# TORlN/HDR-to-SDR

Hardware: AMD Instinct MI355X
Metric: Mpixel/s HDR10->SDR (4K frames) at 1/2/4/8 GPUs; % HBM roofline (higher is better)
Workload: dtype f32

## Files before the change

### hdr-to-sdr_amd/csrc/h2s_tile.h

```cpp
#pragma once
#include "h2s_tile_io.h"

namespace h2s {

__device__ __forceinline__ CurveConsts curve_of(const CurveConsts* frames, int f) {
  typedef __attribute__((address_space(4))) const float cfloat;
  constexpr int n = (int)(sizeof(CurveConsts) / sizeof(float));
  cfloat* src = (cfloat*)frames + __builtin_amdgcn_readfirstlane(f) * n;
  CurveConsts r;
  float* dst = reinterpret_cast<float*>(&r);
#pragma unroll
  for (int i = 0; i < n; i++) dst[i] = src[i];
  return r;
}

constexpr int TILE_WPE = 5;
constexpr int TILE_WPE_LP = TILE_WPE;

template <int TRC, int TM, int DESAT, int LP, int DBG = 0, bool SEMI = false, int SUB = 0>
__global__ __launch_bounds__(256) __attribute__((amdgpu_waves_per_eu(LP ? TILE_WPE_LP : TILE_WPE))) void k_tile(
    const FastParams F) {
  static_assert(DBG == 0 || DBG == 1, "the stage is F.dbg_stage, not a template value");
  static_assert(SUB == 0 || SUB == 3 || (LP == 0 && DBG == 0), "4:2:2 / 4:4:4 input: CPU chain product instances only");
  static_assert(SUB != 3 || (DBG == 0 && SEMI), "top-left 4:2:0 input: the SEMI product instances");
  constexpr bool S420 = SUB == 0 || SUB == 3;
  constexpr int YST = row_stride<LP>(), HST = YST;
  static_assert(TBH * C422_ST <= (CBH + 2) * HST && TBH * C444_ST <= 2 * (CBH + 2) * HST, "hrow holds the SUB windows");
  __shared__ __attribute__((aligned(16))) unsigned char yin[YIN_BYTES];
  __shared__ float hrow[2][(CBH + 2) * HST];
  __shared__ float csum[2][CBH * CBW];
  __shared__ float4 pq_lds[PQ_NSEG + 1];
  __shared__ float4 pqi_lds[LP ? PQI_NTAB : 1];
  extern __shared__ uint16_t eq_lds[];
  __shared__ int tflag[2];
  __shared__ int offtab[4];
  __shared__ unsigned spread_lds[LP ? 256 : 1];
  constexpr int ESC = TRC == 0 || !LP ? PQ_SEG : 1;

  const int t = threadIdx.x;
  const int lane = t & 63, w = t >> 6;
  const unsigned ntiles = F.nbx * F.nby * F.nframes;
  unsigned tile = (unsigned)xcd_remap(blockIdx.x, gridDim.x) * (unsigned)F.tpb;
  const unsigned tend = tile + (unsigned)F.tpb < ntiles ? tile + (unsigned)F.tpb : ntiles;

  TileGeo geo = tile_geo(F, tile);
  const LaneOfs lofs = lane_ofs<SEMI>(F, t);
  TileRegs<SEMI, SUB> cur = tile_load<SEMI, SUB>(F, geo, t, lofs);
  const __amdgpu_buffer_rsrc_t req = __builtin_amdgcn_make_buffer_rsrc((void*)F.eq_lut, (short)0, 2 * F.eq_n, 0x00020000);
  const unsigned eq0 = __builtin_amdgcn_raw_buffer_load_b16(req, 2 * t, 0, 0);
  float4 pq0 = make_float4(0.0f, 0.0f, 0.0f, 0.0f);
  const bool stage_pq = TRC != 1 || !LP || F.lp_ipt;
  if (stage_pq && t < PQ_NSEG) {
    const __amdgpu_buffer_rsrc_t rpq = __builtin_amdgcn_make_buffer_rsrc((void*)F.pq_tab, (short)0, 16 * PQ_NSEG, 0x00020000);
    pq0 = __builtin_bit_cast(float4, __builtin_amdgcn_raw_buffer_load_b128(rpq, 16 * t, 0, 0));
  }
  const int eq_sh = SEMI ? F.out_sh : 0;
  if (t < F.eq_n) eq_lds[t] = (uint16_t)(((eq0 << F.shift_out) | (eq0 >> F.rep_rs)) << eq_sh);
  for (int i = t + 256; i < F.eq_n; i += 256) {
    const unsigned v = __builtin_amdgcn_raw_buffer_load_b16(req, 2 * i, 0, 0);
    eq_lds[i] = (uint16_t)(((v << F.shift_out) | (v >> F.rep_rs)) << eq_sh);
  }
  if (stage_pq && t < PQ_NSEG)
    pq_lds[t + 1] = (TRC == 0 || LP) && t == 0 ? make_float4(0.0f, 0.0f, 3.40282347e38f, 0.0f) : pq0;
  if (stage_pq && t == 255) pq_lds[0] = make_float4(0.0f, 0.0f, 0.0f, 0.0f);
  if (t < 2) tflag[t] = 0;
  if (t < 3) offtab[t] = t == 0 ? 12 : (t == 1 ? F.og : F.ob);
  if (LP) {
    unsigned x = (unsigned)t;
    x = (x | (x << 8)) & 0x0F00Fu;
    x = (x | (x << 4)) & 0x0C30C3u;
    spread_lds[t] = (x | (x << 2)) & 0x249249u;
  }
  __syncthreads();
  if (LP && (F.lp_ipt || TRC == 2)) {
    const __amdgpu_buffer_rsrc_t rpi = __builtin_amdgcn_make_buffer_rsrc((void*)F.pqi_tab, (short)0, 16 * PQI_NTAB, 0x00020000);
    for (int i = t; i < PQI_NTAB; i += 256)
      pqi_lds[i] = __builtin_bit_cast(float4, __builtin_amdgcn_raw_buffer_load_b128(rpi, 16 * i, 0, 0));
  }

  const int qx = (lane >> 2) & 3, qy = lane >> 4, pxl = lane & 1, pyl = (lane >> 1) & 1;
  const int xl = 16 * w + 2 * qx + pxl, yl = 2 * qy + pyl;
  uint16_t* ybase = reinterpret_cast<uint16_t*>(yin + luma_at(xl, yl));
  const float* h0 = hrow[0] + (qy + 1) * HST + xl;
  const float* h1 = hrow[1] + (qy + 1) * HST + xl;
  const int hb = SUB == 3 ? (pyl ? HST : 0) : (pyl ? HST : -HST);
  const float* c0 = hrow[0] + yl * C422_ST + (xl >> 1);
  const float* c1 = hrow[1] + yl * C422_ST + (xl >> 1);
  const int16_t* s0 = reinterpret_cast<const int16_t*>(hrow[0]) + yl * C444_ST + xl;
  const int16_t* s1 = reinterpret_cast<const int16_t*>(hrow[1]) + yl * C444_ST + xl;
  float* csb = csum[0] + qy * CBW + 8 * w + qx;

  const float yoff = in_vgpr(F.y_off_c) * (float)ESC + (ESC == PQ_SEG ? 1.0f : 0.0f);
  const float cmid = in_vgpr(F.c_mid);
  const float a_rv = in_vgpr(F.a_rv[1]) * (float)ESC, a_gv = in_vgpr(F.a_gv[1]) * (float)ESC,
              a_gu = in_vgpr(F.a_gu[1]) * (float)ESC, a_bu = in_vgpr(F.a_bu[1]) * (float)ESC;
  const float stride_g = in_vgpr(F.stride_g), stride_b = in_vgpr(F.stride_b);
  const int og = in_vgpr(F.og), ob = in_vgpr(F.ob), ocr = in_vgpr(F.cr), ocg = in_vgpr(F.cg), ocb = in_vgpr(F.cb);
  const float log2_nm1 = in_vgpr(F.log2_nm1), x_max = in_vgpr(F.x_max);
  const float ysc = in_vgpr(F.ys) * (float)ESC;
  const float ydq = F.dither ? dither_off(xl, yl) - 0.5f : 0.0f;
  const StepK K{a_rv, a_gv, a_gu, a_bu, stride_g, stride_b, og, ob, ocr, ocg, ocb, log2_nm1, x_max,
                TM == 5 && !LP ? in_vgpr(F.hable_kb) : F.hable_kb, F.c111, rintf(1.0f / F.inv_nm1), offtab,
                LP ? in_vgpr(F.lp_k2) : 0.0f, LP ? in_vgpr(F.lp_k2 + 255.0f) : 0.0f, LP ? F.lp_cy + ydq : 0.0f,
                LP ? in_vgpr(F.lp_k1) : 0.0f};
  gu32* lut8v = LP ? in_vgpr64(F.lut8x) : nullptr;
  float qo[4];
#pragma unroll
  for (int i = 0; i < 4; i++)
    qo[i] = LP ? F.lp_qo + (F.lp_dith ? bayer16(xl + 8 * (i & 1), yl + 8 * (i >> 1)) : 0.5f) -
                     (F.lut_off ? 0.0f : F.lp_k2 * F.lp_qs_f)
               : 0.5f;

  auto steps = [&](const TileGeo& g, auto fast) {
    constexpr bool FB = decltype(fast)::value;
    constexpr int YR2 = YROW / 2;
    if constexpr (FB) {
      H2S_MARK("body: fast");
    } else {
      H2S_MARK("body: exact-capable");
    }
    CurveConsts cv = F;
    if ((TM == 7 || TM == 8 || LP) && F.cv_frames) cv = curve_of(F.cv_frames, g.f);
    const CDoviRec* const dv =
        TRC == 2 ? (const CDoviRec*)F.dovi + __builtin_amdgcn_readfirstlane(F.dovi_n == 1 ? 0 : F.dovi_f0 + g.f) : nullptr;
    if constexpr (LP && TM == 7) {
      cv.b_e1b = in_vgpr(cv.b_e1b), cv.b_tb = in_vgpr(cv.b_tb), cv.b_c2 = in_vgpr(cv.b_c2);
      cv.b_lc = in_vgpr(cv.b_lc), cv.b_bk_b = in_vgpr(cv.b_bk_b), cv.b_bk_d = in_vgpr(cv.b_bk_d);
    } else if constexpr (LP && TM == 8) {
      cv.sp_qb_u = in_vgpr(cv.sp_qb_u), cv.sp_pb_u = in_vgpr(cv.sp_pb_u);
      cv.sp_srcmax = in_vgpr(cv.sp_srcmax), cv.sp_umax = in_vgpr(cv.sp_umax);
    }
    const __amdgpu_buffer_rsrc_t lut = __builtin_amdgcn_make_buffer_rsrc((void*)F.lut_yuv, (short)0, F.lut_bytes, 0x00020000);
    const int live = !FB && DBG == 0 && !F.chr444 ? F.H - g.py0 : TBH;
    auto chroma_out = [&](int s, float oyv, float ozv) {
      if (!FB && F.chr444) {
        const int px = g.px0 + xl + 8 * (s & 1), py = g.py0 + yl + 8 * (s >> 1);
        F.chr444[(long long)py * F.chr_w + px] = make_float2(oyv * F.inv_c56, ozv * F.inv_c56);
        return;
      }
      H2S_MARK("S6 chroma quad sums");
      const int oc = 4 * (s >> 1) * CBW + 4 * (s & 1);
      const float su = quad_sum(oyv), sv = quad_sum(ozv);
      csb[oc] = su;
      csb[oc + CBH * CBW] = sv;
    };
    if constexpr (LP && DBG == 0) {
      if (!F.lut_off) {
        unsigned vp = 0;
#pragma unroll
        for (int s = 0; s <= 8; s++) {
          unsigned vn = 0;
          if (s < 8 && (FB || 8 * (s >> 1) < live)) {
            const int oy = 8 * (s >> 1) * YR2 + 8 * (s & 1);
            const int oh = 4 * (s >> 1) * HST + 8 * (s & 1);
            H2S_MARK("S0 step: staged Y, vertical chroma");
            const float ybs = fmaf((float)ybase[oy], ysc, yoff);
            const float U = SUB == 3 ? 2.0f * (h0[oh] + h0[oh + hb]) : fmaf(3.0f, h0[oh], h0[oh + hb]);
            const float V = SUB == 3 ? 2.0f * (h1[oh] + h1[oh + hb]) : fmaf(3.0f, h1[oh], h1[oh + hb]);
            float r, gg, bl;
            lin_tone<TRC, TM, DESAT, LP, 0, FB>(F, cv, pq_lds, pqi_lds, K, ybs, U, V, [](float, float, float) {},
                                                 r, gg, bl, dv);
            H2S_MARK("S3 encode");
            vn = lp_table_read(F, K, lut8v, spread_lds, r, gg, bl, qo[s & 3]);
          }
          if (s > 0 && (FB || 8 * ((s - 1) >> 1) < live)) {
            const int sp = s - 1;
            const float R8 = (float)(vp & 255u), G8 = (float)((vp >> 8) & 255u), B8 = (float)((vp >> 16) & 255u);
            H2S_MARK("S5 Y'CbCr");
            const f3 o = lp_ycbcr(F, K, R8, G8, B8);
            H2S_MARK("S7 eq");
            ybase[8 * (sp >> 1) * YR2 + 8 * (sp & 1)] = eq_lds[(int)o.x];
            chroma_out(sp, o.y, o.z);
          }
          vp = vn;
        }
        return;
      }
      H2S_MARK("body: lut off");
    }
#pragma unroll
    for (int s = 0; s < 8; s++) {
      if (!FB && (s & 1) == 0 && 8 * (s >> 1) >= live) break;
      const int oy = 8 * (s >> 1) * YR2 + 8 * (s & 1);
      const int oh = 4 * (s >> 1) * HST + 8 * (s & 1);
      H2S_MARK("S0 step: staged Y, vertical chroma");
      const float ybs = fmaf((float)ybase[oy], ysc, yoff);
      float U, V;
      if constexpr (SUB == 1) {
        const int oc = 8 * (s >> 1) * C422_ST + 4 * (s & 1);
        U = 4.0f * (c0[oc] + c0[oc + pxl]), V = 4.0f * (c1[oc] + c1[oc + pxl]);
      } else if constexpr (SUB == 2) {
        const int oc = 8 * (s >> 1) * C444_ST + 8 * (s & 1);
        U = 8.0f * (float)s0[oc], V = 8.0f * (float)s1[oc];
      } else if constexpr (SUB == 3) {
        U = 2.0f * (h0[oh] + h0[oh + hb]), V = 2.0f * (h1[oh] + h1[oh + hb]);
      } else {
        U = fmaf(3.0f, h0[oh], h0[oh + hb]);
        V = fmaf(3.0f, h1[oh], h1[oh + hb]);
      }
      const long long di = DBG && g.f == 0 && g.py0 + yl + 8 * (s >> 1) < F.H
                               ? (long long)(g.py0 + yl + 8 * (s >> 1)) * F.dbg_w + g.px0 + xl + 8 * (s & 1)
                               : -1;
      float oyv, ozv;
      ybase[oy] = (uint16_t)px_chain<TRC, TM, DESAT, LP, DBG, FB>(
          F, cv, pq_lds, pqi_lds, eq_lds, lut8v, spread_lds, lut, K, ybs, U, V, di, oyv, ozv, LP ? qo[s & 3] : 0.5f, ydq, dv);
      chroma_out(s, oyv, ozv);
    }
  };
  auto mask_in = [&](uint4& a) {
    a.x &= F.in_mask2, a.y &= F.in_mask2, a.z &= F.in_mask2, a.w &= F.in_mask2;
  };
  auto shift_in = [&](uint4& a) { a.x >>= F.in_sh, a.y >>= F.in_sh, a.z >>= F.in_sh, a.w >>= F.in_sh; };

  const int pl = __builtin_amdgcn_readfirstlane(t >> 6) & 1, rem = t & 63;
  const bool cst = t < 128 && !F.chr444;
  auto commit = [&](unsigned ti) {
    H2S_MARK("tile: commit");
    if constexpr (SEMI && S420) {
      if (!F.in_semi) cur.uh = halo_half(F, geo, t, cur.uh);
    }
    if (F.in_mask2 != 0xFFFFFFFFu) {
      if constexpr (SEMI && S420) {
        if (F.in_sh) {
          shift_in(cur.ya), shift_in(cur.ua);
          cur.uh >>= F.in_sh;
        }
      }
      mask_in(cur.ya), mask_in(cur.ua);
      if constexpr (SUB == 2) mask_in(cur.va);
      else cur.uh &= F.in_mask2;
    }
    const float my = stage_luma(yin, cur.ya, t >> 3, t & 7, ysc, yoff);
    float mc = 0.0f;
    if constexpr (SUB == 1) {
      mc = stage_chroma422(hrow[__builtin_amdgcn_readfirstlane(t >> 7)], cur.ua, cur.uh, t & 127, cmid);
    } else if constexpr (SUB == 2) {
      mc = stage_chroma444(hrow[0], hrow[1], cur.ua, cur.va, t >> 3, t & 7, (int)F.c_mid);
    } else if (SEMI && F.in_semi) {
      if (t < 144) mc = stage_chroma_semi<HST>(hrow[0], hrow[1], cur.ua, cur.uh, t, cmid);
    } else if ((t & 127) < 72) {
      mc = stage_chroma<HST>(hrow[__builtin_amdgcn_readfirstlane(t >> 7)], cur.ua, cur.uh, t & 127, cmid);
    }
    if constexpr (SUB == 2) asm volatile("" ::"v"(cur.ua.w), "v"(cur.va.w));
    else asm volatile("" ::"v"(cur.ua.w), "v"(cur.uh));
    if ((my > F.safe_y || mc > F.safe_c)) tflag[ti & 1u] = 1;
  };
  commit(tile);
  for (;;) {
    H2S_MARK("tile: prefetch");
    const int par = (int)(tile & 1u);
    const TileGeo g = geo;
    const bool more = tile + 1 < tend;
    if (more) {
      tile_next(F, geo);
      cur = tile_load<SEMI, SUB>(F, geo, t, lofs);
    }
    __syncthreads();
    const bool fb = __builtin_amdgcn_readfirstlane(tflag[par]) == 0 && !F.chr444 && !(DBG == 0 && g.py0 + TBH > F.H);
    if (t == 0) tflag[par ^ 1] = 0;
    if (fb)
      steps(g, std::integral_constant<bool, true>{});
    else
      steps(g, std::integral_constant<bool, false>{});
    H2S_MARK("tile: store");
    __syncthreads();

    put_luma(F, g, read_luma(F, yin, t >> 3, t & 7), t >> 3, lofs.sy, t);
    const bool osemi = SEMI && F.out_semi;
    u4v cv{0u, 0u, 0u, 0u};
    int cvo = ST_DROP;
    if (cst) {
      const int cr = osemi ? t >> 3 : rem >> 2;
      cv = osemi ? read_chroma_semi(F, csum[0], cr, t & 7) : read_chroma(F, csum[0], pl, cr, rem & 3);
      if (g.cy0 + cr < F.ch) cvo = lofs.sc;
    }
    put_chroma(F, g, cv, osemi ? 0 : pl, osemi, cvo, t);
    if (!more) break;
    commit(++tile);
  }
}

}
```

### hdr-to-sdr_amd/csrc/h2s_tile_io.h

```cpp
#pragma once
#include "h2s_tile_px.h"

namespace h2s {

constexpr int CBW = 32, CBH = 16;
constexpr int ROW_STRIDE = 72, ROW_STRIDE_LP = 68;
template <int LP>
constexpr int row_stride() { return LP ? ROW_STRIDE_LP : ROW_STRIDE; }
constexpr int AUX_NT = 2;
constexpr int NT = AUX_NT, NTS = AUX_NT;

__device__ __forceinline__ void unpack8(const uint4 a, float* o) {
  o[0] = (float)(a.x & 0xffff), o[1] = (float)(a.x >> 16), o[2] = (float)(a.y & 0xffff), o[3] = (float)(a.y >> 16);
  o[4] = (float)(a.z & 0xffff), o[5] = (float)(a.z >> 16), o[6] = (float)(a.w & 0xffff), o[7] = (float)(a.w >> 16);
}

__device__ __forceinline__ __amdgpu_buffer_rsrc_t plane_rsrc(const uint8_t* base, int bytes) {
  return __builtin_amdgcn_make_buffer_rsrc((void*)base, (short)0, bytes, 0x00020000);
}

template <bool SEMI, int SUB = 0>
struct TileRegs {
  uint4 ya, ua;
  std::conditional_t<SEMI, unsigned, uint16_t> uh;
};
template <bool SEMI>
struct TileRegs<SEMI, 2> {
  uint4 ya, ua, va;
};

struct TileGeo {
  int f, px0, py0, cx0, cy0;
};

__device__ __forceinline__ TileGeo tile_geo(const FastParams& F, unsigned tile) {
  const unsigned bx = tile % F.nbx, bt = tile / F.nbx;
  TileGeo g;
  g.f = (int)(bt / F.nby);
  const int by = (int)(bt % F.nby);
  g.px0 = (int)bx * TBW, g.py0 = by * TBH, g.cx0 = (int)bx * CBW, g.cy0 = by * CBH;
  return g;
}

__device__ __forceinline__ void tile_next(const FastParams& F, TileGeo& g) {
  g.px0 += TBW, g.cx0 += CBW;
  if (g.px0 >= F.W) {
    g.px0 = 0, g.cx0 = 0, g.py0 += TBH, g.cy0 += CBH;
    if (g.py0 >= (int)F.nby * TBH) g.py0 = 0, g.cy0 = 0, g.f++;
  }
}

struct LaneOfs {
  int y, u;
  int sy, sc;
};

template <bool SEMI>
__device__ __forceinline__ LaneOfs lane_ofs(const FastParams& F, int t) {
  LaneOfs L;
  L.y = (t >> 3) * (int)F.in_ls[0] + 16 * (t & 7);
  const int pc = (t >> 7) & 1, tc = t & 127;
  L.u = (tc >> 2) * (int)F.in_ls[1 + pc] + 16 * (tc & 3);
  if (SEMI && F.in_semi) L.u = (t >> 3) * (int)F.in_ls[1] + 16 * (t & 7);
  const int sb = F.out8 ? 8 : 16;
  L.sy = (t >> 3) * (int)F.out_ls[0] + sb * (t & 7);
  const int pl = (t >> 6) & 1, rem = t & 63;
  L.sc = (rem >> 2) * (int)F.out_ls[1 + pl] + sb * (rem & 3);
  if (SEMI && F.out_semi) L.sc = (t >> 3) * (int)F.out_ls[1] + sb * (t & 7);
  return L;
}

template <bool SEMI, int SUB = 0>
__device__ __forceinline__ TileRegs<SEMI, SUB> tile_load(const FastParams& F, const TileGeo& g, int t, const LaneOfs& L) {
  const __amdgpu_buffer_rsrc_t iy = plane_rsrc(F.in[0] + g.f * F.in_fp[0], F.in_bytes[0]);
  const int yr = t >> 3, yc = t & 7;
  TileRegs<SEMI, SUB> r;
  int vy, sy;
  if (g.py0 + TBH <= F.H) {
    vy = L.y, sy = g.py0 * (int)F.in_ls[0] + 2 * g.px0;
  } else {
    vy = (g.py0 + yr < F.H ? g.py0 + yr : F.H - 1) * (int)F.in_ls[0] + 2 * (g.px0 + 8 * yc), sy = 0;
  }
  r.ya = __builtin_bit_cast(uint4, __builtin_amdgcn_raw_buffer_load_b128(iy, vy, sy, NT));
  if constexpr (SUB == 2) {
    const __amdgpu_buffer_rsrc_t iu = plane_rsrc(F.in[1] + g.f * F.in_fp[1], F.in_bytes[1]);
    const __amdgpu_buffer_rsrc_t iv = plane_rsrc(F.in[2] + g.f * F.in_fp[2], F.in_bytes[2]);
    const int lu = (int)F.in_ls[1], lv = (int)F.in_ls[2];
    int vu, vv, su, sv;
    if (g.py0 + TBH <= F.H) {
      vu = yr * lu + 16 * yc, vv = yr * lv + 16 * yc;
      su = g.py0 * lu + 2 * g.px0, sv = g.py0 * lv + 2 * g.px0;
    } else {
      const int row = g.py0 + yr < F.H ? g.py0 + yr : F.H - 1;
      vu = row * lu + 2 * (g.px0 + 8 * yc), vv = row * lv + 2 * (g.px0 + 8 * yc), su = sv = 0;
    }
    r.ua = __builtin_bit_cast(uint4, __builtin_amdgcn_raw_buffer_load_b128(iu, vu, su, NT));
    r.va = __builtin_bit_cast(uint4, __builtin_amdgcn_raw_buffer_load_b128(iv, vv, sv, NT));
    return r;
  } else if constexpr (SUB == 1) {
    const int pc = __builtin_amdgcn_readfirstlane(t >> 7), tc = t & 127;
    const __amdgpu_buffer_rsrc_t ic = plane_rsrc(F.in[1 + pc] + g.f * F.in_fp[1 + pc], F.in_bytes[1 + pc]);
    const int ls = (int)F.in_ls[1 + pc];
    int vc, vh, sc;
    if (g.py0 + TBH <= F.H && g.cx0 + CBW + 1 <= F.icw) {
      vc = L.u, vh = L.u + 16, sc = g.py0 * ls + 2 * g.cx0;
    } else {
      const int clr = tc >> 2, ccx = tc & 3;
      const int row = g.py0 + clr < F.H ? g.py0 + clr : F.H - 1;
      vc = row * ls + 2 * (g.cx0 + 8 * ccx);
      vh = row * ls + 2 * chroma_edge_at(g.cx0 + 8 * ccx + 8, F.icw, F.chroma_edge);
      sc = 0;
    }
    if ((tc & 3) != 3) vh = 0x7FFFFFF0;
    r.ua = __builtin_bit_cast(uint4, __builtin_amdgcn_raw_buffer_load_b128(ic, vc, sc, NT));
    r.uh = __builtin_amdgcn_raw_buffer_load_b16(ic, vh, sc, 0);
    return r;
  } else {
  const bool pair = SEMI && F.in_semi;
  int pc, vc, vh, sc;
  if (pair) {
    pc = 0;
    const int ls = (int)F.in_ls[1];
    if (g.cy0 >= 1 && g.cy0 + CBH + 1 <= F.ch && g.cx0 + CBW + 1 <= F.cw) {
      vc = L.u, vh = L.u + 16, sc = (g.cy0 - 1) * ls + 4 * g.cx0;
    } else {
      const int clr = t >> 3, ccx = t & 7;
      const int row = chroma_edge_at(g.cy0 - 1 + clr, F.ch, F.chroma_edge);
      vc = row * ls + 4 * (g.cx0 + 4 * ccx);
      vh = row * ls + 4 * chroma_edge_at(g.cx0 + 4 * ccx + 4, F.cw, F.chroma_edge);
      sc = 0;
    }
    if (t >= 144) vc = vh = 0x7FFFFFF0;
  } else {
    pc = __builtin_amdgcn_readfirstlane(t >> 7);
    const int tc = t & 127;
    const int ls = (int)F.in_ls[1 + pc];
    if (g.cy0 >= 1 && g.cy0 + CBH + 1 <= F.ch && g.cx0 + CBW + 1 <= F.cw) {
      vc = L.u, vh = L.u + 16, sc = (g.cy0 - 1) * ls + 2 * g.cx0;
    } else {
      const int clr = tc >> 2, ccx = tc & 3;
      const int row = chroma_edge_at(g.cy0 - 1 + clr, F.ch, F.chroma_edge);
      vc = row * ls + 2 * (g.cx0 + 8 * ccx);
      vh = row * ls + 2 * chroma_edge_at(g.cx0 + 8 * ccx + 8, F.cw, F.chroma_edge);
      sc = 0;
    }
    if (tc >= 72) vc = vh = 0x7FFFFFF0;
  }
  const __amdgpu_buffer_rsrc_t ic = plane_rsrc(F.in[1 + pc] + g.f * F.in_fp[1 + pc], F.in_bytes[1 + pc]);
  sc = __builtin_amdgcn_readfirstlane(sc);
  r.ua = __builtin_bit_cast(uint4, __builtin_amdgcn_raw_buffer_load_b128(ic, vc, sc, NT));
  if constexpr (SEMI) {
    r.uh = __builtin_amdgcn_raw_buffer_load_b32(ic, vh & ~2, sc, 0);
  } else {
    r.uh = __builtin_amdgcn_raw_buffer_load_b16(ic, vh, sc, 0);
  }
  return r;
  }
}

__device__ __forceinline__ unsigned halo_half(const FastParams& F, const TileGeo& g, int t, unsigned hw) {
  int hs = 0;
  if (!(g.cy0 >= 1 && g.cy0 + CBH + 1 <= F.ch && g.cx0 + CBW + 1 <= F.cw))
    hs = (chroma_edge_at(g.cx0 + 8 * (t & 3) + 8, F.cw, F.chroma_edge) & 1) << 4;
  return (hw >> hs) & 0xffffu;
}

constexpr int YROW = 144;
constexpr int luma_at(int x, int y) { return y * YROW + 2 * x; }
static_assert(YROW % 16 == 0 && luma_at(8, 0) == 16, "a chunk of 8 samples is one aligned 16-byte slot");
static_assert(luma_at(0, 1) >= luma_at(TBW - 1, 0) + 2, "the rows' slots are disjoint");
static_assert((luma_at(0, 1) / 4) % 32 == 4 && luma_at(7, 0) / 4 == 3, "a step's 8 rows x 4 dwords cover the 32 banks once");
constexpr int YIN_BYTES = luma_at(0, TBH);
typedef unsigned short us2v __attribute__((ext_vector_type(2)));
__device__ __forceinline__ float stage_luma(unsigned char* yin, uint4 a, int row, int col8, float ysc, float yoff) {
  *reinterpret_cast<uint4*>(yin + luma_at(8 * col8, row)) = a;
  const us2v m = __builtin_elementwise_max(
      __builtin_elementwise_max(__builtin_bit_cast(us2v, a.x), __builtin_bit_cast(us2v, a.y)),
      __builtin_elementwise_max(__builtin_bit_cast(us2v, a.z), __builtin_bit_cast(us2v, a.w)));
  return fmaf((float)(m.x > m.y ? m.x : m.y), ysc, yoff);
}
template <int HST>
__device__ __forceinline__ float stage_chroma(float* plane, uint4 a, unsigned h, int tt, float cmid) {
  float v[9];
  unpack8(a, v);
  v[8] = (float)h;
#pragma unroll
  for (int k = 0; k < 9; k++) v[k] -= cmid;
  float m = fabsf(v[0]);
#pragma unroll
  for (int k = 1; k < 9; k++) m = __builtin_fmaxf(m, fabsf(v[k]));
  float* d = plane + (tt >> 2) * HST + 16 * (tt & 3);
#pragma unroll
  for (int k = 0; k < 4; k++)
    *reinterpret_cast<float4*>(d + 4 * k) =
        make_float4(v[2 * k] + v[2 * k], v[2 * k] + v[2 * k + 1], v[2 * k + 1] + v[2 * k + 1], v[2 * k + 1] + v[2 * k + 2]);
  return m;
}
template <int HST>
__device__ __forceinline__ float stage_chroma_semi(float* plane_u, float* plane_v, uint4 a, unsigned h, int tt, float cmid) {
  const unsigned w[5] = {a.x, a.y, a.z, a.w, h};
  float u[5], v[5];
#pragma unroll
  for (int k = 0; k < 5; k++) u[k] = (float)(w[k] & 0xffff) - cmid, v[k] = (float)(w[k] >> 16) - cmid;
  float m = __builtin_fmaxf(fabsf(u[0]), fabsf(v[0]));
#pragma unroll
  for (int k = 1; k < 5; k++) m = __builtin_fmaxf(m, __builtin_fmaxf(fabsf(u[k]), fabsf(v[k])));
  const int o = (tt >> 3) * HST + 8 * (tt & 7);
#pragma unroll
  for (int k = 0; k < 2; k++) {
    *reinterpret_cast<float4*>(plane_u + o + 4 * k) =
        make_float4(u[2 * k] + u[2 * k], u[2 * k] + u[2 * k + 1], u[2 * k + 1] + u[2 * k + 1], u[2 * k + 1] + u[2 * k + 2]);
    *reinterpret_cast<float4*>(plane_v + o + 4 * k) =
        make_float4(v[2 * k] + v[2 * k], v[2 * k] + v[2 * k + 1], v[2 * k + 1] + v[2 * k + 1], v[2 * k + 1] + v[2 * k + 2]);
  }
  return m;
}
constexpr int C422_ST = 36;
constexpr int C444_ST = 72;
__device__ __forceinline__ float stage_chroma422(float* plane, uint4 a, unsigned h, int tt, float cmid) {
  float v[9];
  unpack8(a, v);
  v[8] = (float)h;
#pragma unroll
  for (int k = 0; k < 9; k++) v[k] -= cmid;
  float m = fabsf(v[0]);
#pragma unroll
  for (int k = 1; k < 8; k++) m = __builtin_fmaxf(m, fabsf(v[k]));
  float* d = plane + (tt >> 2) * C422_ST + 8 * (tt & 3);
  *reinterpret_cast<float4*>(d) = make_float4(v[0], v[1], v[2], v[3]);
  *reinterpret_cast<float4*>(d + 4) = make_float4(v[4], v[5], v[6], v[7]);
  if ((tt & 3) == 3) d[8] = v[8], m = __builtin_fmaxf(m, fabsf(v[8]));
  return m;
}
__device__ __forceinline__ float stage_chroma444(float* plane_u, float* plane_v, uint4 a, uint4 b, int row, int col8,
                                                 int imid) {
  auto pack = [&](uint4 q, float* plane, float& m) {
    const unsigned w[4] = {q.x, q.y, q.z, q.w};
    unsigned o[4];
#pragma unroll
    for (int k = 0; k < 4; k++) {
      const int lo = (int)(w[k] & 0xffff) - imid, hi = (int)(w[k] >> 16) - imid;
      m = __builtin_fmaxf(m, __builtin_fmaxf(fabsf((float)lo), fabsf((float)hi)));
      o[k] = ((unsigned)lo & 0xffffu) | ((unsigned)hi << 16);
    }
    *reinterpret_cast<uint4*>(reinterpret_cast<int16_t*>(plane) + row * C444_ST + 8 * col8) = make_uint4(o[0], o[1], o[2], o[3]);
  };
  float m = 0.0f;
  pack(a, plane_u, m);
  pack(b, plane_v, m);
  return m;
}
__device__ __forceinline__ u4v read_luma(const FastParams& F, const unsigned char* yin, int r, int c) {
  const uint4 a = *reinterpret_cast<const uint4*>(yin + luma_at(8 * c, r));
  if (F.out8)
    return u4v{__builtin_amdgcn_perm(a.y, a.x, 0x06040200u), __builtin_amdgcn_perm(a.w, a.z, 0x06040200u), 0u, 0u};
  return u4v{a.x, a.y, a.z, a.w};
}
constexpr int ST_DROP = (int)0x80000000u;
__device__ __forceinline__ void tile_store(const FastParams& F, u4v v, __amdgpu_buffer_rsrc_t rs, int vo, int so, int t) {
  if (F.out8) {
    v.z = (unsigned)__builtin_amdgcn_update_dpp(0, (int)v.x, 0xB1, 0xF, 0xF, false);
    v.w = (unsigned)__builtin_amdgcn_update_dpp(0, (int)v.y, 0xB1, 0xF, 0xF, false);
    if (t & 1) vo = ST_DROP;
  }
  __builtin_amdgcn_raw_buffer_store_b128(v, rs, vo, so, NTS);
}
__device__ __forceinline__ void put_luma(const FastParams& F, const TileGeo& g, u4v v, int r, int vo, int t) {
  if (g.py0 + r >= F.H) vo = ST_DROP;
  const __amdgpu_buffer_rsrc_t oy_ = plane_rsrc(F.out[0] + g.f * F.out_fp[0], F.out_bytes[0]);
  tile_store(F, v, oy_, vo, g.py0 * (int)F.out_ls[0] + (F.out8 ? g.px0 : 2 * g.px0), t);
}
__device__ __forceinline__ u4v read_chroma(const FastParams& F, const float* csum, int pl, int r, int c) {
  const float4* src = reinterpret_cast<const float4*>(csum + pl * (CBH * CBW) + r * CBW + 8 * c);
  const float4 v0 = src[0], v1 = src[1];
  const float vv[8] = {v0.x, v0.y, v0.z, v0.w, v1.x, v1.y, v1.z, v1.w};
  unsigned code[8];
  if (F.dither) {
#pragma unroll
    for (int k = 0; k < 8; k++) code[k] = (unsigned)(int)(vv[k] + (F.c_bias - 0.5f + dither_off(k, r)));
  } else {
#pragma unroll
    for (int k = 0; k < 8; k++) code[k] = (unsigned)(int)(vv[k] + F.c_bias);
  }
  if (F.rep_rs == 31) {
#pragma unroll
    for (int k = 0; k < 8; k++) code[k] <<= F.shift_out;
  } else {
#pragma unroll
    for (int k = 0; k < 8; k++) code[k] = (code[k] << F.shift_out) | (code[k] >> F.rep_rs);
  }
  if (F.out8)
    return u4v{code[0] | (code[1] << 8) | (code[2] << 16) | (code[3] << 24),
               code[4] | (code[5] << 8) | (code[6] << 16) | (code[7] << 24), 0u, 0u};
  return u4v{code[0] | (code[1] << 16), code[2] | (code[3] << 16), code[4] | (code[5] << 16), code[6] | (code[7] << 16)};
}
__device__ __forceinline__ void put_chroma(const FastParams& F, const TileGeo& g, u4v v, int pl, bool semi, int vo, int t) {
  const __amdgpu_buffer_rsrc_t oc_ = plane_rsrc(F.out[1 + pl] + g.f * F.out_fp[1 + pl], F.out_bytes[1 + pl]);
  tile_store(F, v, oc_, vo, g.cy0 * (int)F.out_ls[1 + pl] + ((F.out8 ? g.cx0 : 2 * g.cx0) << (semi ? 1 : 0)), t);
}

__device__ __forceinline__ u4v read_chroma_semi(const FastParams& F, const float* csum, int r, int c) {
  const float4 vu = *reinterpret_cast<const float4*>(csum + r * CBW + 4 * c);
  const float4 vv = *reinterpret_cast<const float4*>(csum + CBH * CBW + r * CBW + 4 * c);
  const float s[8] = {vu.x, vv.x, vu.y, vv.y, vu.z, vv.z, vu.w, vv.w};
  unsigned code[8];
  if (F.dither) {
#pragma unroll
    for (int k = 0; k < 8; k++) code[k] = (unsigned)(int)(s[k] + (F.c_bias - 0.5f + dither_off(4 * (c & 1) + (k >> 1), r)));
  } else {
#pragma unroll
    for (int k = 0; k < 8; k++) code[k] = (unsigned)(int)(s[k] + F.c_bias);
  }
  if (F.rep_rs == 31) {
#pragma unroll
    for (int k = 0; k < 8; k++) code[k] <<= F.shift_out;
  } else {
#pragma unroll
    for (int k = 0; k < 8; k++) code[k] = (code[k] << F.shift_out) | (code[k] >> F.rep_rs);
  }
  if (F.out8)
    return u4v{code[0] | (code[1] << 8) | (code[2] << 16) | (code[3] << 24),
               code[4] | (code[5] << 8) | (code[6] << 16) | (code[7] << 24), 0u, 0u};
  return u4v{(code[0] | (code[1] << 16)) << F.out_sh, (code[2] | (code[3] << 16)) << F.out_sh,
             (code[4] | (code[5] << 16)) << F.out_sh, (code[6] | (code[7] << 16)) << F.out_sh};
}

}
```

Measured before the change: 280,100.

## Carry per-tile plane descriptors across tiles and pack frame pitches into a lane bank

Plane origins, line strides and byte sizes are now computed once into a TilePlanes struct and advanced only when the frame changes. Frame pitches, the scratch pointer and chroma constants are parked in one VGPR (one value per lane) and read back with readlane, which is meant to cut scalar register pressure and per-tile kernarg loads. Chroma tile coordinates are derived from the luma coordinates instead of being stored, and the rep_rs==31 special case is dropped. The waves-per-EU attribute gains an explicit upper bound. The risks are extra readlane and s_nop overhead and possible register-allocation shifts.

New measurement: 281,600, median of 5. No clear change (+0.5%).

```diff
diff --git a/hdr-to-sdr_amd/csrc/h2s_tile.h b/hdr-to-sdr_amd/csrc/h2s_tile.h
--- a/hdr-to-sdr_amd/csrc/h2s_tile.h
+++ b/hdr-to-sdr_amd/csrc/h2s_tile.h
@@ -15,16 +15,18 @@
 }
 
 constexpr int TILE_WPE = 5;
+constexpr int TILE_WPE_MAX = 5;
 constexpr int TILE_WPE_LP = TILE_WPE;
 
 template <int TRC, int TM, int DESAT, int LP, int DBG = 0, bool SEMI = false, int SUB = 0>
-__global__ __launch_bounds__(256) __attribute__((amdgpu_waves_per_eu(LP ? TILE_WPE_LP : TILE_WPE))) void k_tile(
+__global__ __launch_bounds__(256) __attribute__((amdgpu_waves_per_eu(LP ? TILE_WPE_LP : TILE_WPE, LP ? 8 : TILE_WPE_MAX))) void k_tile(
     const FastParams F) {
   static_assert(DBG == 0 || DBG == 1, "the stage is F.dbg_stage, not a template value");
   static_assert(SUB == 0 || SUB == 3 || (LP == 0 && DBG == 0), "4:2:2 / 4:4:4 input: CPU chain product instances only");
   static_assert(SUB != 3 || (DBG == 0 && SEMI), "top-left 4:2:0 input: the SEMI product instances");
   constexpr bool S420 = SUB == 0 || SUB == 3;
   constexpr int YST = row_stride<LP>(), HST = YST;
+  constexpr bool CARRY = !LP && !DBG && TM != 7 && TM != 8;
   static_assert(TBH * C422_ST <= (CBH + 2) * HST && TBH * C444_ST <= 2 * (CBH + 2) * HST, "hrow holds the SUB windows");
   __shared__ __attribute__((aligned(16))) unsigned char yin[YIN_BYTES];
   __shared__ float hrow[2][(CBH + 2) * HST];
@@ -44,8 +46,9 @@
   const unsigned tend = tile + (unsigned)F.tpb < ntiles ? tile + (unsigned)F.tpb : ntiles;
 
   TileGeo geo = tile_geo(F, tile);
-  const LaneOfs lofs = lane_ofs<SEMI>(F, t);
-  TileRegs<SEMI, SUB> cur = tile_load<SEMI, SUB>(F, geo, t, lofs);
+  TilePlanes planes = tile_planes<SEMI, SUB, CARRY>(F, geo, t);
+  const LaneOfs lofs = lane_ofs<SEMI>(F, planes, t);
+  TileRegs<SEMI, SUB> cur = tile_load<SEMI, SUB>(F, planes, geo, t, lofs);
   const __amdgpu_buffer_rsrc_t req = __builtin_amdgcn_make_buffer_rsrc((void*)F.eq_lut, (short)0, 2 * F.eq_n, 0x00020000);
   const unsigned eq0 = __builtin_amdgcn_raw_buffer_load_b16(req, 2 * t, 0, 0);
   float4 pq0 = make_float4(0.0f, 0.0f, 0.0f, 0.0f);
@@ -131,11 +134,17 @@
       cv.sp_srcmax = in_vgpr(cv.sp_srcmax), cv.sp_umax = in_vgpr(cv.sp_umax);
     }
     const __amdgpu_buffer_rsrc_t lut = __builtin_amdgcn_make_buffer_rsrc((void*)F.lut_yuv, (short)0, F.lut_bytes, 0x00020000);
-    const int live = !FB && DBG == 0 && !F.chr444 ? F.H - g.py0 : TBH;
+    const int live = !FB && DBG == 0 && !planes.is(IO_SCRATCH) ? F.H - g.py0 : TBH;
     auto chroma_out = [&](int s, float oyv, float ozv) {
-      if (!FB && F.chr444) {
+      if (!FB && planes.is(IO_SCRATCH)) {
         const int px = g.px0 + xl + 8 * (s & 1), py = g.py0 + yl + 8 * (s >> 1);
-        F.chr444[(long long)py * F.chr_w + px] = make_float2(oyv * F.inv_c56, ozv * F.inv_c56);
+        const float inv_c56 = CARRY ? __int_as_float(planes.bank.get(BK_INV_C56)) : F.inv_c56;
+        const int chr_w = CARRY ? planes.bank.get(BK_CHR_W) : F.chr_w;
+        const long long scratch = CARRY ? planes.bank.get64(BK_SCRATCH) : (long long)F.chr444;
+        typedef float f2v __attribute__((ext_vector_type(2)));
+        typedef __attribute__((address_space(1))) f2v gf2v;
+        ((gf2v*)scratch)[(long long)py * chr_w + px] =
+            f2v{oyv * inv_c56, ozv * inv_c56};
         return;
       }
       H2S_MARK("S6 chroma quad sums");
@@ -213,13 +222,13 @@
   auto shift_in = [&](uint4& a) { a.x >>= F.in_sh, a.y >>= F.in_sh, a.z >>= F.in_sh, a.w >>= F.in_sh; };
 
   const int pl = __builtin_amdgcn_readfirstlane(t >> 6) & 1, rem = t & 63;
-  const bool cst = t < 128 && !F.chr444;
+  const int crole = t < 128 && !F.chr444;
   auto commit = [&](unsigned ti) {
     H2S_MARK("tile: commit");
     if constexpr (SEMI && S420) {
       if (!F.in_semi) cur.uh = halo_half(F, geo, t, cur.uh);
     }
-    if (F.in_mask2 != 0xFFFFFFFFu) {
+    if (planes.is(IO_MASK)) {
       if constexpr (SEMI && S420) {
         if (F.in_sh) {
           shift_in(cur.ya), shift_in(cur.ua);
@@ -249,14 +258,16 @@
   for (;;) {
     H2S_MARK("tile: prefetch");
     const int par = (int)(tile & 1u);
+    planes.bank.keep();
     const TileGeo g = geo;
     const bool more = tile + 1 < tend;
     if (more) {
-      tile_next(F, geo);
-      cur = tile_load<SEMI, SUB>(F, geo, t, lofs);
+      tile_next<SUB, CARRY>(F, geo, planes);
+      if constexpr (!CARRY) planes = tile_planes<SEMI, SUB, CARRY>(F, geo, t);
+      cur = tile_load<SEMI, SUB>(F, planes, geo, t, lofs);
     }
     __syncthreads();
-    const bool fb = __builtin_amdgcn_readfirstlane(tflag[par]) == 0 && !F.chr444 && !(DBG == 0 && g.py0 + TBH > F.H);
+    const bool fb = __builtin_amdgcn_readfirstlane(tflag[par]) == 0 && !planes.is(IO_SCRATCH) && !(DBG == 0 && g.py0 + TBH > F.H);
     if (t == 0) tflag[par ^ 1] = 0;
     if (fb)
       steps(g, std::integral_constant<bool, true>{});
@@ -265,17 +276,21 @@
     H2S_MARK("tile: store");
     __syncthreads();
 
-    put_luma(F, g, read_luma(F, yin, t >> 3, t & 7), t >> 3, lofs.sy, t);
+    if constexpr (!CARRY) planes = tile_planes<SEMI, SUB, CARRY>(F, g, t);
+    put_luma(F, planes, g, read_luma(planes, yin, t >> 3, t & 7), t >> 3, lofs.sy);
     const bool osemi = SEMI && F.out_semi;
     u4v cv{0u, 0u, 0u, 0u};
     int cvo = ST_DROP;
-    if (cst) {
+    if (crole) {
       const int cr = osemi ? t >> 3 : rem >> 2;
-      cv = osemi ? read_chroma_semi(F, csum[0], cr, t & 7) : read_chroma(F, csum[0], pl, cr, rem & 3);
-      if (g.cy0 + cr < F.ch) cvo = lofs.sc;
-    }
-    put_chroma(F, g, cv, osemi ? 0 : pl, osemi, cvo, t);
+      cv = osemi ? read_chroma_semi(F, planes, csum[0], cr, t & 7) : read_chroma(F, planes, csum[0], pl, cr, rem & 3);
+      if (g.cy0() + cr < F.ch) cvo = lofs.sc;
+    }
+    put_chroma(F, planes, g, cv, osemi, cvo);
     if (!more) break;
+    if constexpr (CARRY) {
+      if (geo.f != g.f) out_next_frame(planes);
+    }
     commit(++tile);
   }
 }
diff --git a/hdr-to-sdr_amd/csrc/h2s_tile_io.h b/hdr-to-sdr_amd/csrc/h2s_tile_io.h
--- a/hdr-to-sdr_amd/csrc/h2s_tile_io.h
+++ b/hdr-to-sdr_amd/csrc/h2s_tile_io.h
@@ -30,62 +30,142 @@
 };
 
 struct TileGeo {
-  int f, px0, py0, cx0, cy0;
-};
+  int f, px0, py0;
+  __device__ __forceinline__ int cx0() const { return px0 >> 1; }
+  __device__ __forceinline__ int cy0() const { return py0 >> 1; }
+};
+static_assert(TBW == 2 * CBW && TBH == 2 * CBH, "TileGeo::cx0, cy0");
 
 __device__ __forceinline__ TileGeo tile_geo(const FastParams& F, unsigned tile) {
   const unsigned bx = tile % F.nbx, bt = tile / F.nbx;
   TileGeo g;
   g.f = (int)(bt / F.nby);
   const int by = (int)(bt % F.nby);
-  g.px0 = (int)bx * TBW, g.py0 = by * TBH, g.cx0 = (int)bx * CBW, g.cy0 = by * CBH;
+  g.px0 = (int)bx * TBW, g.py0 = by * TBH;
   return g;
 }
 
-__device__ __forceinline__ void tile_next(const FastParams& F, TileGeo& g) {
-  g.px0 += TBW, g.cx0 += CBW;
+struct PlaneRef {
+  const uint8_t* org;
+  int ls, bytes;
+};
+__device__ __forceinline__ int uniform(int x) { return __builtin_amdgcn_readfirstlane(x); }
+__device__ __forceinline__ long long uniform(long long x) {
+  return (long long)(((unsigned long long)(unsigned)uniform((int)((unsigned long long)x >> 32)) << 32) |
+                     (unsigned)uniform((int)x));
+}
+struct LaneBank {
+  int v, lane;
+  __device__ __forceinline__ void put(int k, int x) { v = lane == k ? x : v; }
+  __device__ __forceinline__ void put64(int k, long long x) { put(k, (int)x), put(k + 1, (int)((unsigned long long)x >> 32)); }
+  __device__ __forceinline__ int get(int k) const { return __builtin_amdgcn_readlane(v, k); }
+  __device__ __forceinline__ long long get64(int k) const {
+    return (long long)(((unsigned long long)(unsigned)get(k + 1) << 32) | (unsigned)get(k));
+  }
+  __device__ __forceinline__ void keep() { asm volatile("" : "+v"(v)); }
+};
+enum : int { BK_IY_FP = 0, BK_IC_FP = 2, BK_IV_FP = 4, BK_OY_FP = 6, BK_OC_FP = 8, BK_SCRATCH = 10, BK_CHR_W = 12, BK_INV_C56 = 13 };
+enum : int { IO_OUT8 = 1, IO_DITHER = 2, IO_MASK = 4, IO_SCRATCH = 8 };
+
+struct TilePlanes {
+  PlaneRef iy, ic, iv, oy, oc;
+  int osh, flags;
+  LaneBank bank;
+  __device__ __forceinline__ bool is(int bit) const {
+    int f = flags;
+    asm volatile("" : "+s"(f));
+    return (f & bit) != 0;
+  }
+};
+__device__ __forceinline__ PlaneRef plane_ref(const uint8_t* const* base, const long long* ls, const long long* fp,
+                                              const int* bytes, int p, int f, LaneBank& bank, int k) {
+  PlaneRef r;
+  const long long pitch = uniform(fp[p]);
+  if (k >= 0) bank.put64(k, pitch);
+  r.org = (const uint8_t*)uniform((long long)(base[p] + f * pitch));
+  r.ls = uniform((int)ls[p]), r.bytes = uniform(bytes[p]);
+  return r;
+}
+template <bool SEMI, int SUB, bool CARRY>
+__device__ __forceinline__ TilePlanes tile_planes(const FastParams& F, const TileGeo& g, int t) {
+  TilePlanes P;
+  P.bank.v = 0, P.bank.lane = t & 63;
+  constexpr int BK_IY_FP = CARRY ? h2s::BK_IY_FP : -1, BK_IC_FP = CARRY ? h2s::BK_IC_FP : -1, BK_IV_FP = CARRY ? h2s::BK_IV_FP : -1,
+                BK_OY_FP = CARRY ? h2s::BK_OY_FP : -1, BK_OC_FP = CARRY ? h2s::BK_OC_FP : -1;
+  const int pc = SUB == 2 || (SEMI && SUB != 1 && F.in_semi) ? 0 : uniform(t >> 7);
+  const int pl = SEMI && F.out_semi ? 0 : uniform(t >> 6) & 1;
+  P.iy = plane_ref(F.in, F.in_ls, F.in_fp, F.in_bytes, 0, g.f, P.bank, BK_IY_FP);
+  P.ic = plane_ref(F.in, F.in_ls, F.in_fp, F.in_bytes, 1 + pc, g.f, P.bank, BK_IC_FP);
+  P.iv = SUB == 2 ? plane_ref(F.in, F.in_ls, F.in_fp, F.in_bytes, 2, g.f, P.bank, BK_IV_FP) : P.ic;
+  P.oy = plane_ref(F.out, F.out_ls, F.out_fp, F.out_bytes, 0, g.f, P.bank, BK_OY_FP);
+  P.oc = plane_ref(F.out, F.out_ls, F.out_fp, F.out_bytes, 1 + pl, g.f, P.bank, BK_OC_FP);
+  if constexpr (CARRY) {
+    P.bank.put64(BK_SCRATCH, (long long)F.chr444);
+    P.bank.put(BK_CHR_W, F.chr_w), P.bank.put(BK_INV_C56, __float_as_int(F.inv_c56));
+  }
+  P.osh = uniform(F.out8 ? 0 : 1);
+  P.flags = uniform((F.out8 ? IO_OUT8 : 0) | (F.dither ? IO_DITHER : 0) | (F.in_mask2 != 0xFFFFFFFFu ? IO_MASK : 0) |
+                    (F.chr444 ? IO_SCRATCH : 0));
+  return P;
+}
+
+template <int SUB, bool CARRY>
+__device__ __forceinline__ void tile_next(const FastParams& F, TileGeo& g, TilePlanes& P) {
+  g.px0 += TBW;
   if (g.px0 >= F.W) {
-    g.px0 = 0, g.cx0 = 0, g.py0 += TBH, g.cy0 += CBH;
-    if (g.py0 >= (int)F.nby * TBH) g.py0 = 0, g.cy0 = 0, g.f++;
-  }
+    g.px0 = 0, g.py0 += TBH;
+    if (g.py0 >= (int)F.nby * TBH) {
+      g.py0 = 0, g.f++;
+      if constexpr (CARRY) {
+        P.iy.org += P.bank.get64(BK_IY_FP), P.ic.org += P.bank.get64(BK_IC_FP);
+        if constexpr (SUB == 2) P.iv.org += P.bank.get64(BK_IV_FP);
+      }
+    }
+  }
+}
+__device__ __forceinline__ void out_next_frame(TilePlanes& P) {
+  P.oy.org += P.bank.get64(BK_OY_FP), P.oc.org += P.bank.get64(BK_OC_FP);
 }
 
 struct LaneOfs {
   int y, u;
   int sy, sc;
 };
+constexpr int ST_DROP = (int)0x80000000u;
 
 template <bool SEMI>
-__device__ __forceinline__ LaneOfs lane_ofs(const FastParams& F, int t) {
+__device__ __forceinline__ LaneOfs lane_ofs(const FastParams& F, const TilePlanes& P, int t) {
   LaneOfs L;
-  L.y = (t >> 3) * (int)F.in_ls[0] + 16 * (t & 7);
-  const int pc = (t >> 7) & 1, tc = t & 127;
-  L.u = (tc >> 2) * (int)F.in_ls[1 + pc] + 16 * (tc & 3);
-  if (SEMI && F.in_semi) L.u = (t >> 3) * (int)F.in_ls[1] + 16 * (t & 7);
-  const int sb = F.out8 ? 8 : 16;
-  L.sy = (t >> 3) * (int)F.out_ls[0] + sb * (t & 7);
-  const int pl = (t >> 6) & 1, rem = t & 63;
-  L.sc = (rem >> 2) * (int)F.out_ls[1 + pl] + sb * (rem & 3);
-  if (SEMI && F.out_semi) L.sc = (t >> 3) * (int)F.out_ls[1] + sb * (t & 7);
+  L.y = (t >> 3) * P.iy.ls + 16 * (t & 7);
+  const int tc = t & 127;
+  L.u = (tc >> 2) * P.ic.ls + 16 * (tc & 3);
+  if (SEMI && F.in_semi) L.u = (t >> 3) * P.ic.ls + 16 * (t & 7);
+  const int sb = 8 << P.osh;
+  L.sy = (t >> 3) * P.oy.ls + sb * (t & 7);
+  const int rem = t & 63;
+  L.sc = (rem >> 2) * P.oc.ls + sb * (rem & 3);
+  if (SEMI && F.out_semi) L.sc = (t >> 3) * P.oc.ls + sb * (t & 7);
+  if (F.out8 && (t & 1)) L.sy = L.sc = ST_DROP;
   return L;
 }
 
 template <bool SEMI, int SUB = 0>
-__device__ __forceinline__ TileRegs<SEMI, SUB> tile_load(const FastParams& F, const TileGeo& g, int t, const LaneOfs& L) {
-  const __amdgpu_buffer_rsrc_t iy = plane_rsrc(F.in[0] + g.f * F.in_fp[0], F.in_bytes[0]);
+__device__ __forceinline__ TileRegs<SEMI, SUB> tile_load(const FastParams& F, const TilePlanes& P, const TileGeo& g, int t,
+                                                         const LaneOfs& L) {
+  const __amdgpu_buffer_rsrc_t iy = plane_rsrc(P.iy.org, P.iy.bytes);
   const int yr = t >> 3, yc = t & 7;
   TileRegs<SEMI, SUB> r;
   int vy, sy;
   if (g.py0 + TBH <= F.H) {
-    vy = L.y, sy = g.py0 * (int)F.in_ls[0] + 2 * g.px0;
-  } else {
-    vy = (g.py0 + yr < F.H ? g.py0 + yr : F.H - 1) * (int)F.in_ls[0] + 2 * (g.px0 + 8 * yc), sy = 0;
+    vy = L.y, sy = g.py0 * P.iy.ls + 2 * g.px0;
+  } else {
+    vy = (g.py0 + yr < F.H ? g.py0 + yr : F.H - 1) * P.iy.ls + 2 * (g.px0 + 8 * yc), sy = 0;
   }
   r.ya = __builtin_bit_cast(uint4, __builtin_amdgcn_raw_buffer_load_b128(iy, vy, sy, NT));
   if constexpr (SUB == 2) {
-    const __amdgpu_buffer_rsrc_t iu = plane_rsrc(F.in[1] + g.f * F.in_fp[1], F.in_bytes[1]);
-    const __amdgpu_buffer_rsrc_t iv = plane_rsrc(F.in[2] + g.f * F.in_fp[2], F.in_bytes[2]);
-    const int lu = (int)F.in_ls[1], lv = (int)F.in_ls[2];
+    const __amdgpu_buffer_rsrc_t iu = plane_rsrc(P.ic.org, P.ic.bytes);
+    const __amdgpu_buffer_rsrc_t iv = plane_rsrc(P.iv.org, P.iv.bytes);
+    const int lu = P.ic.ls, lv = P.iv.ls;
     int vu, vv, su, sv;
     if (g.py0 + TBH <= F.H) {
       vu = yr * lu + 16 * yc, vv = yr * lv + 16 * yc;
@@ -98,17 +178,17 @@
     r.va = __builtin_bit_cast(uint4, __builtin_amdgcn_raw_buffer_load_b128(iv, vv, sv, NT));
     return r;
   } else if constexpr (SUB == 1) {
-    const int pc = __builtin_amdgcn_readfirstlane(t >> 7), tc = t & 127;
-    const __amdgpu_buffer_rsrc_t ic = plane_rsrc(F.in[1 + pc] + g.f * F.in_fp[1 + pc], F.in_bytes[1 + pc]);
-    const int ls = (int)F.in_ls[1 + pc];
+    const int tc = t & 127;
+    const __amdgpu_buffer_rsrc_t ic = plane_rsrc(P.ic.org, P.ic.bytes);
+    const int ls = P.ic.ls;
     int vc, vh, sc;
-    if (g.py0 + TBH <= F.H && g.cx0 + CBW + 1 <= F.icw) {
-      vc = L.u, vh = L.u + 16, sc = g.py0 * ls + 2 * g.cx0;
+    if (g.py0 + TBH <= F.H && g.cx0() + CBW + 1 <= F.icw) {
+      vc = L.u, vh = L.u + 16, sc = g.py0 * ls + 2 * g.cx0();
     } else {
       const int clr = tc >> 2, ccx = tc & 3;
       const int row = g.py0 + clr < F.H ? g.py0 + clr : F.H - 1;
-      vc = row * ls + 2 * (g.cx0 + 8 * ccx);
-      vh = row * ls + 2 * chroma_edge_at(g.cx0 + 8 * ccx + 8, F.icw, F.chroma_edge);
+      vc = row * ls + 2 * (g.cx0() + 8 * ccx);
+      vh = row * ls + 2 * chroma_edge_at(g.cx0() + 8 * ccx + 8, F.icw, F.chroma_edge);
       sc = 0;
     }
     if ((tc & 3) != 3) vh = 0x7FFFFFF0;
@@ -117,36 +197,33 @@
     return r;
   } else {
   const bool pair = SEMI && F.in_semi;
-  int pc, vc, vh, sc;
+  const int ls = P.ic.ls;
+  int vc, vh, sc;
   if (pair) {
-    pc = 0;
-    const int ls = (int)F.in_ls[1];
-    if (g.cy0 >= 1 && g.cy0 + CBH + 1 <= F.ch && g.cx0 + CBW + 1 <= F.cw) {
-      vc = L.u, vh = L.u + 16, sc = (g.cy0 - 1) * ls + 4 * g.cx0;
+    if (g.cy0() >= 1 && g.cy0() + CBH + 1 <= F.ch && g.cx0() + CBW + 1 <= F.cw) {
+      vc = L.u, vh = L.u + 16, sc = (g.cy0() - 1) * ls + 4 * g.cx0();
     } else {
       const int clr = t >> 3, ccx = t & 7;
-      const int row = chroma_edge_at(g.cy0 - 1 + clr, F.ch, F.chroma_edge);
-      vc = row * ls + 4 * (g.cx0 + 4 * ccx);
-      vh = row * ls + 4 * chroma_edge_at(g.cx0 + 4 * ccx + 4, F.cw, F.chroma_edge);
+      const int row = chroma_edge_at(g.cy0() - 1 + clr, F.ch, F.chroma_edge);
+      vc = row * ls + 4 * (g.cx0() + 4 * ccx);
+      vh = row * ls + 4 * chroma_edge_at(g.cx0() + 4 * ccx + 4, F.cw, F.chroma_edge);
       sc = 0;
     }
     if (t >= 144) vc = vh = 0x7FFFFFF0;
   } else {
-    pc = __builtin_amdgcn_readfirstlane(t >> 7);
     const int tc = t & 127;
-    const int ls = (int)F.in_ls[1 + pc];
-    if (g.cy0 >= 1 && g.cy0 + CBH + 1 <= F.ch && g.cx0 + CBW + 1 <= F.cw) {
-      vc = L.u, vh = L.u + 16, sc = (g.cy0 - 1) * ls + 2 * g.cx0;
+    if (g.cy0() >= 1 && g.cy0() + CBH + 1 <= F.ch && g.cx0() + CBW + 1 <= F.cw) {
+      vc = L.u, vh = L.u + 16, sc = (g.cy0() - 1) * ls + 2 * g.cx0();
     } else {
       const int clr = tc >> 2, ccx = tc & 3;
-      const int row = chroma_edge_at(g.cy0 - 1 + clr, F.ch, F.chroma_edge);
-      vc = row * ls + 2 * (g.cx0 + 8 * ccx);
-      vh = row * ls + 2 * chroma_edge_at(g.cx0 + 8 * ccx + 8, F.cw, F.chroma_edge);
+      const int row = chroma_edge_at(g.cy0() - 1 + clr, F.ch, F.chroma_edge);
+      vc = row * ls + 2 * (g.cx0() + 8 * ccx);
+      vh = row * ls + 2 * chroma_edge_at(g.cx0() + 8 * ccx + 8, F.cw, F.chroma_edge);
       sc = 0;
     }
     if (tc >= 72) vc = vh = 0x7FFFFFF0;
   }
-  const __amdgpu_buffer_rsrc_t ic = plane_rsrc(F.in[1 + pc] + g.f * F.in_fp[1 + pc], F.in_bytes[1 + pc]);
+  const __amdgpu_buffer_rsrc_t ic = plane_rsrc(P.ic.org, P.ic.bytes);
   sc = __builtin_amdgcn_readfirstlane(sc);
   r.ua = __builtin_bit_cast(uint4, __builtin_amdgcn_raw_buffer_load_b128(ic, vc, sc, NT));
   if constexpr (SEMI) {
@@ -160,8 +237,8 @@
 
 __device__ __forceinline__ unsigned halo_half(const FastParams& F, const TileGeo& g, int t, unsigned hw) {
   int hs = 0;
-  if (!(g.cy0 >= 1 && g.cy0 + CBH + 1 <= F.ch && g.cx0 + CBW + 1 <= F.cw))
-    hs = (chroma_edge_at(g.cx0 + 8 * (t & 3) + 8, F.cw, F.chroma_edge) & 1) << 4;
+  if (!(g.cy0() >= 1 && g.cy0() + CBH + 1 <= F.ch && g.cx0() + CBW + 1 <= F.cw))
+    hs = (chroma_edge_at(g.cx0() + 8 * (t & 3) + 8, F.cw, F.chroma_edge) & 1) << 4;
   return (hw >> hs) & 0xffffu;
 }
 
@@ -250,75 +327,62 @@
   pack(b, plane_v, m);
   return m;
 }
-__device__ __forceinline__ u4v read_luma(const FastParams& F, const unsigned char* yin, int r, int c) {
+__device__ __forceinline__ u4v read_luma(const TilePlanes& P, const unsigned char* yin, int r, int c) {
   const uint4 a = *reinterpret_cast<const uint4*>(yin + luma_at(8 * c, r));
-  if (F.out8)
+  if (P.is(IO_OUT8))
     return u4v{__builtin_amdgcn_perm(a.y, a.x, 0x06040200u), __builtin_amdgcn_perm(a.w, a.z, 0x06040200u), 0u, 0u};
   return u4v{a.x, a.y, a.z, a.w};
 }
-constexpr int ST_DROP = (int)0x80000000u;
-__device__ __forceinline__ void tile_store(const FastParams& F, u4v v, __amdgpu_buffer_rsrc_t rs, int vo, int so, int t) {
-  if (F.out8) {
+__device__ __forceinline__ void tile_store(const TilePlanes& P, u4v v, __amdgpu_buffer_rsrc_t rs, int vo, int so) {
+  if (P.is(IO_OUT8)) {
     v.z = (unsigned)__builtin_amdgcn_update_dpp(0, (int)v.x, 0xB1, 0xF, 0xF, false);
     v.w = (unsigned)__builtin_amdgcn_update_dpp(0, (int)v.y, 0xB1, 0xF, 0xF, false);
-    if (t & 1) vo = ST_DROP;
-  }
-  __builtin_amdgcn_raw_buffer_store_b128(v, rs, vo, so, NTS);
-}
-__device__ __forceinline__ void put_luma(const FastParams& F, const TileGeo& g, u4v v, int r, int vo, int t) {
+  }
+  __builtin_amdgcn_raw_buffer_store_b128(v, rs, vo, uniform(so), NTS);
+  asm volatile("s_nop 15" ::"v"(v.x), "v"(v.y), "v"(v.z), "v"(v.w));
+}
+__device__ __forceinline__ void put_luma(const FastParams& F, const TilePlanes& P, const TileGeo& g, u4v v, int r, int vo) {
   if (g.py0 + r >= F.H) vo = ST_DROP;
-  const __amdgpu_buffer_rsrc_t oy_ = plane_rsrc(F.out[0] + g.f * F.out_fp[0], F.out_bytes[0]);
-  tile_store(F, v, oy_, vo, g.py0 * (int)F.out_ls[0] + (F.out8 ? g.px0 : 2 * g.px0), t);
-}
-__device__ __forceinline__ u4v read_chroma(const FastParams& F, const float* csum, int pl, int r, int c) {
+  tile_store(P, v, plane_rsrc(P.oy.org, P.oy.bytes), vo, g.py0 * P.oy.ls + (g.px0 << P.osh));
+}
+__device__ __forceinline__ u4v read_chroma(const FastParams& F, const TilePlanes& P, const float* csum, int pl, int r, int c) {
   const float4* src = reinterpret_cast<const float4*>(csum + pl * (CBH * CBW) + r * CBW + 8 * c);
   const float4 v0 = src[0], v1 = src[1];
   const float vv[8] = {v0.x, v0.y, v0.z, v0.w, v1.x, v1.y, v1.z, v1.w};
   unsigned code[8];
-  if (F.dither) {
+  if (P.is(IO_DITHER)) {
 #pragma unroll
     for (int k = 0; k < 8; k++) code[k] = (unsigned)(int)(vv[k] + (F.c_bias - 0.5f + dither_off(k, r)));
   } else {
 #pragma unroll
     for (int k = 0; k < 8; k++) code[k] = (unsigned)(int)(vv[k] + F.c_bias);
   }
-  if (F.rep_rs == 31) {
-#pragma unroll
-    for (int k = 0; k < 8; k++) code[k] <<= F.shift_out;
-  } else {
-#pragma unroll
-    for (int k = 0; k < 8; k++) code[k] = (code[k] << F.shift_out) | (code[k] >> F.rep_rs);
-  }
-  if (F.out8)
+#pragma unroll
+  for (int k = 0; k < 8; k++) code[k] = (code[k] << F.shift_out) | (code[k] >> F.rep_rs);
+  if (P.is(IO_OUT8))
     return u4v{code[0] | (code[1] << 8) | (code[2] << 16) | (code[3] << 24),
                code[4] | (code[5] << 8) | (code[6] << 16) | (code[7] << 24), 0u, 0u};
   return u4v{code[0] | (code[1] << 16), code[2] | (code[3] << 16), code[4] | (code[5] << 16), code[6] | (code[7] << 16)};
 }
-__device__ __forceinline__ void put_chroma(const FastParams& F, const TileGeo& g, u4v v, int pl, bool semi, int vo, int t) {
-  const __amdgpu_buffer_rsrc_t oc_ = plane_rsrc(F.out[1 + pl] + g.f * F.out_fp[1 + pl], F.out_bytes[1 + pl]);
-  tile_store(F, v, oc_, vo, g.cy0 * (int)F.out_ls[1 + pl] + ((F.out8 ? g.cx0 : 2 * g.cx0) << (semi ? 1 : 0)), t);
-}
-
-__device__ __forceinline__ u4v read_chroma_semi(const FastParams& F, const float* csum, int r, int c) {
+__device__ __forceinline__ void put_chroma(const FastParams& F, const TilePlanes& P, const TileGeo& g, u4v v, bool semi, int vo) {
+  tile_store(P, v, plane_rsrc(P.oc.org, P.oc.bytes), vo, g.cy0() * P.oc.ls + ((g.cx0() << P.osh) << (semi ? 1 : 0)));
+}
+
+__device__ __forceinline__ u4v read_chroma_semi(const FastParams& F, const TilePlanes& P, const float* csum, int r, int c) {
   const float4 vu = *reinterpret_cast<const float4*>(csum + r * CBW + 4 * c);
   const float4 vv = *reinterpret_cast<const float4*>(csum + CBH * CBW + r * CBW + 4 * c);
   const float s[8] = {vu.x, vv.x, vu.y, vv.y, vu.z, vv.z, vu.w, vv.w};
   unsigned code[8];
-  if (F.dither) {
+  if (P.is(IO_DITHER)) {
 #pragma unroll
     for (int k = 0; k < 8; k++) code[k] = (unsigned)(int)(s[k] + (F.c_bias - 0.5f + dither_off(4 * (c & 1) + (k >> 1), r)));
   } else {
 #pragma unroll
     for (int k = 0; k < 8; k++) code[k] = (unsigned)(int)(s[k] + F.c_bias);
   }
-  if (F.rep_rs == 31) {
-#pragma unroll
-    for (int k = 0; k < 8; k++) code[k] <<= F.shift_out;
-  } else {
-#pragma unroll
-    for (int k = 0; k < 8; k++) code[k] = (code[k] << F.shift_out) | (code[k] >> F.rep_rs);
-  }
-  if (F.out8)
+#pragma unroll
+  for (int k = 0; k < 8; k++) code[k] = (code[k] << F.shift_out) | (code[k] >> F.rep_rs);
+  if (P.is(IO_OUT8))
     return u4v{code[0] | (code[1] << 8) | (code[2] << 16) | (code[3] << 24),
                code[4] | (code[5] << 8) | (code[6] << 16) | (code[7] << 24), 0u, 0u};
   return u4v{(code[0] | (code[1] << 16)) << F.out_sh, (code[2] | (code[3] << 16)) << F.out_sh,
```
